# maomaomi1/Mean-Field-Multi-Agent-Reinforcement-Learning

Measured on NVIDIA B200. Metric: battle agent-steps/sec incl. obs+mean-action, higher is better.
Workload: dtype f32

## Files before the change

mean-field-multi-agent-reinforcement-learning_b200/csrc/battle_kernels.cuh:

```cuda
#pragma once
#include <cuda_runtime.h>
#include <stdint.h>

#include "battle_types.h"
#include "rng.cuh"

namespace mfmarl {

__device__ __forceinline__ int pos_x(int p) { return p & 0xFFFF; }
__device__ __forceinline__ int pos_y(int p) { return (p >> 16) & 0xFFFF; }
__device__ __forceinline__ int pack_pos(int x, int y) { return (x & 0xFFFF) | (y << 16); }
__device__ __forceinline__ uint32_t st_dead(uint32_t s) { return s & 1u; }
__device__ __forceinline__ uint32_t st_op(uint32_t s) { return (s >> 8) & 0xFFu; }
__device__ __forceinline__ uint32_t st_act(uint32_t s) { return (s >> 16) & 0xFFu; }
__device__ __forceinline__ uint32_t st_with_op(uint32_t s, uint32_t op) { return (s & ~0xFF00u) | (op << 8); }
__device__ __forceinline__ uint32_t make_state(uint32_t dead, uint32_t op, uint32_t act) {
    return dead | (op << 8) | (act << 16);
}

__device__ __forceinline__ int block_scan_flags2(bool fa, bool fb, int *s_warp, int &total) {
    const unsigned ba = __ballot_sync(0xFFFFFFFFu, fa), bb = __ballot_sync(0xFFFFFFFFu, fb);
    const int lane = threadIdx.x & 31, w = threadIdx.x >> 5;
    if (lane == 0) s_warp[w] = __popc(ba) | (__popc(bb) << 16);
    __syncthreads();
// ... 33 lines not shown
    R.hp10 = ((W + 2 * kPad) * (H + 2 * kPad) * 2 + 15) & ~15;
    R.mini = R.hp10 + 4 * 2 * cap;
    R.total = (R.mini + 4 * 2 * kViewCells + 15) & ~15;
    return R;
}

__device__ __forceinline__ void build_obs_record(const BattleParams &P, const BattleState &S, int e, uint16_t *s_pg, int *s_cnt) {
    const int tid = threadIdx.x, nt = blockDim.x, W = P.W, cap = P.cap, PW = W + 2 * kPad;
    const ObsRecord R = obs_record_layout(P.W, P.H, cap);
    unsigned char *rec = S.obs_record + (size_t)e * R.total;
    const size_t ebase = (size_t)e * 2 * cap;
    for (int c = tid; c < R.hp10 / 16; c += nt) ((uint4 *)s_pg)[c] = ((const uint4 *)S.grid_template)[c];
    for (int c = tid; c < 2 * kViewCells; c += nt) s_cnt[c] = 0;
    const int n0 = S.num[e * 2], n1 = S.num[e * 2 + 1];
    __syncthreads();
    const uint8_t *lut = S.mini_lut;
    float *hp10 = (float *)(rec + R.hp10);
    for (int s = tid; s < 2 * cap; s += nt) {
        const int gg = s >= cap, i = s - gg * cap;
        if (i >= (gg ? n1 : n0)) continue;
        const int p = S.pos[ebase + s], x = pos_x(p), y = pos_y(p);
        atomicAdd(&s_cnt[gg * kViewCells + lut[W + y] + lut[x]], 1);
        if (!st_dead(S.state[ebase + s])) {
            s_pg[(y + kPad) * PW + x + kPad] = (uint16_t)(((2 + gg) << 14) | s);
            hp10[s] = __fdiv_rn(S.hp[ebase + s], P.hp);
        }
    }
    __syncthreads();
    for (int c = tid; c < R.hp10 / 16; c += nt) ((uint4 *)rec)[c] = ((const uint4 *)s_pg)[c];
    float *mini = (float *)(rec + R.mini);
    for (int c = tid; c < 2 * kViewCells; c += nt) {
        const int tot = c >= kViewCells ? n1 : n0;
        mini[c] = tot > 0 ? __fdiv_rn((float)s_cnt[c], (float)tot) : 0.0f;
    }
}

__device__ __forceinline__ void place_from_template(const BattleParams &P, const BattleState &S, int e, int side) {
    const int cap = P.cap, n_action = P.n_move + P.n_attack;
    const size_t ebase = (size_t)e * 2 * cap;
    const int32_t *tpos = S.init_pos + (size_t)e * P.tmpl_stride;
    const int32_t *tnum = S.init_num + (P.tmpl_stride ? 2 * e : 0);
    for (int s = threadIdx.x; s < 2 * cap; s += blockDim.x) {
        const int g = s >= cap, i = s - g * cap, src = (side ? 1 - g : g) * cap + i;
        const bool live = i < tnum[side ? 1 - g : g];
        S.pos[ebase + s] = live ? tpos[src] : 0;
        S.hp[ebase + s] = P.hp;
        S.id[ebase + s] = live ? tpos[2 * cap + src] : 0;
        S.state[ebase + s] = make_state(0, OP_NULL, (uint32_t)n_action);
        S.next_rew[ebase + s] = P.step_reward;
        S.last_rew[ebase + s] = 0.0f;
    }
    if (threadIdx.x < 2) { S.num[e * 2 + threadIdx.x] = tnum[side ? 1 - threadIdx.x : threadIdx.x]; S.dead_ct[e * 2 + threadIdx.x] = 0; }
    if (threadIdx.x == 0) { S.step_ct[e] = 0; S.id_counter[e] = tnum[0] + tnum[1]; S.side[e] = side; }
}

__device__ __forceinline__ uint32_t minstd_jump(uint32_t s, uint32_t n) {
    const uint32_t pw[12] = {16807u, 282475249u, 984943658u, 1457850878u, 1137522503u, 1636807826u,
                             685118024u, 515204530u, 897054849u, 2038299453u, 1836275591u, 349037107u};
    uint64_t acc = s;
#pragma unroll
    for (int b = 0; b < 12; b++)
        if ((n >> b) & 1u) acc = (acc * pw[b]) % 2147483647ull;
    return (uint32_t)acc;
}

struct StepSmem {
    int pos, hp, nr, state, att, aux, mv, mvt, tag_a, tag_v, mvidx, scr0, scr1, grid, misc, total;
};
__host__ __device__ inline StepSmem step_smem_layout(int W, int H, int cap, int obs_cached) {
    StepSmem L;
    const int n = 2 * cap;
    int o = 0;
    L.pos = o;   o += 4 * n;
    L.hp = o;    o += 4 * n;
    L.nr = o;    o += 4 * n;
    L.state = o; o += 4 * n;
    L.att = o;   o += 4 * n;
    L.aux = o;   o += 4 * n;
    L.mv = o;    o += 4 * n;
    L.mvt = o;   o += 4 * n;
    L.scr0 = o;  o += 4 * n;
    L.scr1 = o;  o += 4 * n;
    L.tag_a = o; o += 2 * n;
    L.tag_v = o; o += 2 * n;
    L.mvidx = o; o += 2 * n;
    L.misc = o;  o += 4 * 128;
    L.grid = o;
    {
        int bytes = 4 * W * H;
        const int need = obs_record_layout(W, H, cap).hp10 + 4 * 2 * kViewCells;
        if (obs_cached && need > bytes) bytes = need;
        o += (bytes + 15) & ~15;
    }
    L.total = (o + 15) & ~15;
    return L;
}

enum { MISC_WARP = 0, MISC_N = 32, MISC_DEAD = 34, MISC_FLAG = 40, MISC_HIST = 64 };

enum : int { MV_FAIL = 0, MV_OK = 1, MV_WAIT = 2 };

__global__ void k_step(const __grid_constant__ BattleParams P, const BattleState S, const StepIO io) {
    extern __shared__ __align__(128) unsigned char smem_raw[];
    const StepSmem L = step_smem_layout(P.W, P.H, P.cap, P.obs_cached);
    int *s_pos = (int *)(smem_raw + L.pos);
    float *s_hp = (float *)(smem_raw + L.hp);
    float *s_nr = (float *)(smem_raw + L.nr);
    uint32_t *s_state = (uint32_t *)(smem_raw + L.state);
    uint32_t *s_att = (uint32_t *)(smem_raw + L.att);
    int *s_aux = (int *)(smem_raw + L.aux);
    uint32_t *s_mv = (uint32_t *)(smem_raw + L.mv);
    int *s_mvt = (int *)(smem_raw + L.mvt);
    int *s_scr0 = (int *)(smem_raw + L.scr0);
    int *s_scr1 = (int *)(smem_raw + L.scr1);
    uint16_t *s_tag_a = (uint16_t *)(smem_raw + L.tag_a);
    uint16_t *s_tag_v = (uint16_t *)(smem_raw + L.tag_v);
    uint16_t *s_mvidx = (uint16_t *)(smem_raw + L.mvidx);
    int *s_misc = (int *)(smem_raw + L.misc);
    uint32_t *s_grid = (uint32_t *)(smem_raw + L.grid);
    constexpr uint32_t kNoClaim = 0xFFFF0000u;

    const int e = blockIdx.x, tid = threadIdx.x, nt = blockDim.x;
    const int cap = P.cap, W = P.W, H = P.H, cells = W * H;
    const int n_action = P.n_move + P.n_attack;
    const size_t ebase = (size_t)e * 2 * cap;
    const int phases = io.phases;
    const int step_before = S.step_ct[e];

    if (tid < 2) { s_misc[MISC_N + tid] = S.num[e * 2 + tid]; s_misc[MISC_DEAD + tid] = S.dead_ct[e * 2 + tid]; }
    const uint8_t *walls = S.walls + (size_t)e * P.wall_stride;
    if ((cells & 3) == 0) {
        for (int c = tid; c < (cells >> 2); c += nt) {
            const uint32_t w4 = ((const uint32_t *)walls)[c];
            ((uint4 *)s_grid)[c] = make_uint4(kNoClaim | (w4 & 0xFFu), kNoClaim | ((w4 >> 8) & 0xFFu),
                                              kNoClaim | ((w4 >> 16) & 0xFFu), kNoClaim | (w4 >> 24));
        }
    } else {
        for (int c = tid; c < cells; c += nt) s_grid[c] = kNoClaim | walls[c];
    }
    __syncthreads();
    const int n0 = s_misc[MISC_N], n1 = s_misc[MISC_N + 1];
    for (int s = tid; s < 2 * cap; s += nt) {
        const int g = s >= cap, i = s - g * cap;
        if (i < (g ? n1 : n0)) {
            const int p = S.pos[ebase + s];
            uint32_t st = S.state[ebase + s];
            if ((phases & PH_SETACT) && ((io.setact_mask >> g) & 1)) {
                int a = io.actions[ebase + s];
                a = (a < 0 || a >= n_action) ? n_action : a;
                st = (st & 0xFF00FFFFu) | ((uint32_t)a << 16);
            }
            s_pos[s] = p; s_hp[s] = S.hp[ebase + s]; s_nr[s] = S.next_rew[ebase + s];
            s_state[s] = st;
            if (!st_dead(st)) s_grid[pos_y(p) * W + pos_x(p)] = kNoClaim | (uint32_t)(2 + s);
        }
        s_tag_a[s] = 0; s_tag_v[s] = 0; s_mvidx[s] = 0; s_scr0[s] = 0;
    }
    __syncthreads();

    int done = 0;
    if (phases & PH_STEP) {
        int nA = 0, nM = 0;
        const int n_pass = P.move_bands > 0 ? P.move_bands + 1 : 1;
        for (int pass = 0; pass < n_pass; pass++) {
            for (int gi = 0; gi < kGroups; gi++) {
                const int g = io.group_seq[gi];
                if (g < 0) continue;
                const int ng = g ? n1 : n0;
                for (int base = 0; base < ng; base += nt) {
                    const int i = base + tid, s = g * cap + i;
                    const bool valid = i < ng;
                    const int a = valid ? (int)st_act(s_state[s]) : n_action;
                    bool is_mv = valid && a < P.n_move;
                    const bool is_at = pass == 0 && valid && a >= P.n_move && a < n_action;
                    if (is_mv && n_pass > 1) {
                        const int x = pos_x(s_pos[s]), xr = x % P.band_width;
// ... 280 lines not shown
        __syncthreads();
        if (P.random_sides) {
            const uint4 r = philox4x32_10(make_uint4((uint32_t)episode, 0x51DEu, 0u, 0u), make_uint2(P.seed, (uint32_t)(P.env_base + e)));
            side = (int)(r.x & 1u);
        }
        place_from_template(P, S, e, side);
        if (tid == 0) S.episode[e] = episode;
    } else if (phases & PH_CLEAR) {
        for (int g = 0; g < kGroups; g++) {
            const int ng = g ? n1 : n0;
            int kept = 0;
            for (int base = 0; base < ng; base += nt) {
                const int i = base + tid, s = g * cap + i;
                const bool keep = i < ng && !st_dead(s_state[s]);
                const int my_id = keep ? S.id[ebase + s] : 0;
                int tot;
                const int p = block_scan_flag(keep, s_misc + MISC_WARP, tot);
                if (keep) {
                    const size_t d = ebase + (size_t)g * cap + kept + p;
                    S.pos[d] = s_pos[s]; S.hp[d] = s_hp[s]; S.id[d] = my_id;
                    S.state[d] = make_state(0, OP_NULL, st_act(s_state[s]));
                    S.last_rew[d] = s_nr[s];
                    S.next_rew[d] = P.step_reward;
                }
                kept += tot;
            }
            if (tid == 0) { S.num[e * 2 + g] = kept; S.dead_ct[e * 2 + g] = 0; }
        }
    } else if (phases & (PH_STEP | PH_SETACT)) {
        for (int s = tid; s < 2 * cap; s += nt) {
            const int g = s >= cap, i = s - g * cap;
            if (i < (g ? n1 : n0)) {
                S.pos[ebase + s] = s_pos[s]; S.hp[ebase + s] = s_hp[s];
                S.state[ebase + s] = s_state[s]; S.next_rew[ebase + s] = s_nr[s];
            }
        }
        if (tid < 2) S.dead_ct[e * 2 + tid] = s_misc[MISC_DEAD + tid];
    }
    if (io.mirror.pos != nullptr) {
        __syncthreads();
        for (int s = tid; s < 2 * cap; s += nt) {
            io.mirror.pos[s] = S.pos[ebase + s]; io.mirror.id[s] = S.id[ebase + s]; io.mirror.state[s] = S.state[ebase + s];
            io.mirror.hp[s] = S.hp[ebase + s]; io.mirror.next_rew[s] = S.next_rew[ebase + s];
            io.mirror.last_rew[s] = S.last_rew[ebase + s];
        }
        if (tid < 2) { io.mirror.head[tid] = S.num[e * 2 + tid]; io.mirror.head[2 + tid] = S.dead_ct[e * 2 + tid]; }
        if (tid == 0) { io.mirror.head[4] = done; io.mirror.head[5] = S.step_ct[e]; }
    }
    if (P.obs_cached && (phases & (PH_STEP | PH_CLEAR))) {
        __syncthreads();
        build_obs_record(P, S, e, (uint16_t *)(smem_raw + L.grid),
                         (int *)(smem_raw + L.grid + obs_record_layout(P.W, P.H, P.cap).hp10));
    }
}

__global__ void k_obs_record(const __grid_constant__ BattleParams P, const BattleState S) {
    extern __shared__ __align__(128) unsigned char smem_raw[];
    build_obs_record(P, S, blockIdx.x, (uint16_t *)smem_raw, (int *)(smem_raw + obs_record_layout(P.W, P.H, P.cap).hp10));
}

#ifndef MF_OBS_CHUNK
#define MF_OBS_CHUNK 8
#endif
constexpr int kObsChunk = MF_OBS_CHUNK;
constexpr int kObsThreads = 32 * kObsChunk, kObsWarps = kObsThreads / 32;
constexpr int kObsCtasPerSm = 16 / kObsChunk;
constexpr int kObsStageBytes = kObsChunk * kViewRow * 4;
constexpr int kViewRowBf16Bytes = kViewCells * 16;
constexpr int kObsPasses = (kViewCells + 31) / 32;
static_assert(kObsChunk == kObsWarps, "one warp composes one row of a chunk");

struct ObsSmem { int stage0, stage1, rec, hp10, mini, cnt, code, fxy, tmpl, record, total; };
constexpr int kObsMaxTile = kObsThreads;
__host__ __device__ inline bool obs_template_in_smem(int W, int H) { return (W + 2 * kPad) * (H + 2 * kPad) * 2 <= 8 * 1024; }
__host__ __device__ inline ObsSmem obs_smem_layout(int W, int H, int cap, int cached, int bf16 = 0) {
    ObsSmem L; int o = 0;
    const int stage_bytes = bf16 ? kObsChunk * kViewRowBf16Bytes : kObsStageBytes;
    L.stage0 = o; o += stage_bytes;
    L.stage1 = o; o += stage_bytes;
    L.rec = o;    o += 16 * kObsMaxTile;
    L.record = L.cnt = L.tmpl = 0;
    if (cached) {
        const ObsRecord R = obs_record_layout(W, H, cap);
        L.record = o; L.code = o + R.grid; L.hp10 = o + R.hp10; L.mini = o + R.mini; o += R.total;
        L.fxy = o;    o += 4 * (W + H);
        o = (o + 15) & ~15;
    } else {
        L.hp10 = o;   o += 4 * 2 * cap;
        L.mini = o;   o += 4 * 2 * kViewCells;
        L.cnt = o;    o += 4 * 2 * kViewCells;
        L.code = o;   o += (2 * (W + 2 * kPad) * (H + 2 * kPad) + 3) & ~3;
        L.fxy = o;    o += 4 * (W + H);
        o = (o + 15) & ~15;
        L.tmpl = o;   if (obs_template_in_smem(W, H)) o += (2 * (W + 2 * kPad) * (H + 2 * kPad) + 15) & ~15;
    }
    L.total = (o + 127) & ~127;
    return L;
}

__device__ __forceinline__ void bulk_store_s2g(void *gdst, const void *ssrc, uint32_t bytes) {
    const uint32_t saddr = (uint32_t)__cvta_generic_to_shared(ssrc);
    asm volatile("cp.async.bulk.global.shared::cta.bulk_group [%0], [%1], %2;"
                 :: "l"(gdst), "r"(saddr), "r"(bytes) : "memory");
}
__device__ __forceinline__ void bulk_commit() { asm volatile("cp.async.bulk.commit_group;" ::: "memory"); }
template <int N> __device__ __forceinline__ void bulk_wait_read() {
// ... 20 lines not shown
    extern __shared__ __align__(128) unsigned char smem_raw[];
    const ObsSmem L = obs_smem_layout(P.W, P.H, P.cap, CACHED, BF16);
    constexpr int kRowBytes = BF16 ? kViewRowBf16Bytes : kViewRow * 4;
    constexpr int kStageBytes = kObsChunk * kRowBytes;
    float *const s_stage0 = (float *)(smem_raw + L.stage0), *const s_stage1 = (float *)(smem_raw + L.stage1);
    int4 *s_rec = (int4 *)(smem_raw + L.rec);
    float *s_hp10 = (float *)(smem_raw + L.hp10);
    float *s_mini = (float *)(smem_raw + L.mini);
    int *s_cnt = (int *)(smem_raw + L.cnt);
    uint16_t *s_code = (uint16_t *)(smem_raw + L.code);
    float *s_fxy = (float *)(smem_raw + L.fxy);
    const bool tmpl_smem = !CACHED && obs_template_in_smem(P.W, P.H);
    const uint4 *s_tmpl = tmpl_smem ? (const uint4 *)(smem_raw + L.tmpl) : (const uint4 *)S.grid_template;
    const uint32_t rec_bytes = (uint32_t)obs_record_layout(P.W, P.H, P.cap).total;

    const int tid = threadIdx.x, lane = tid & 31, warp = tid >> 5;
    const int W = P.W, H = P.H, cap = P.cap;
    const int PW = W + 2 * kPad, pcells = PW * (H + 2 * kPad);
    const int FS = P.feature_size, emb = P.embedding_size, n_action = P.n_move + P.n_attack;
    const uint8_t *lut = S.mini_lut;

    constexpr int kDiscPasses = kObsDiscSlots / 32;
    int off[kDiscPasses], cell7[kDiscPasses];
#pragma unroll
    for (int it = 0; it < kDiscPasses; it++) {
        const int c = P.obs_cell[it * 32 + lane];
        const int vy = c / kView, vx = c - vy * kView;
        off[it] = c < kViewCells ? vy * PW + vx : 0;
        cell7[it] = c < kViewCells ? c * kChan : -1;
    }
    for (int i = tid; i < 2 * kStageBytes / 16; i += kObsThreads) ((uint4 *)s_stage0)[i] = make_uint4(0u, 0u, 0u, 0u);
    if (tmpl_smem)
        for (int c = tid; c < (pcells * 2 + 15) / 16; c += kObsThreads)
            ((uint4 *)(smem_raw + L.tmpl))[c] = ((const uint4 *)S.grid_template)[c];
    for (int i = tid; i < W + H; i += kObsThreads)
        s_fxy[i] = i < W ? __fdiv_rn((float)i, (float)W) : __fdiv_rn((float)(i - W), (float)H);

    int buf = 0;
    const int groups_per_env = io.group_mask == 3 ? 2 : 1;
    const int n_items = P.E * groups_per_env * io.tiles_per_group;
    __shared__ int s_next;
    if (tid == 0) s_next = atomicAdd(&S.obs_ticket[0], 1);
    for (;;) {
        __syncthreads();
        const int item = s_next;
        __syncthreads();
        if (item >= n_items) break;
        int next_ticket = 0;
        if (tid == 0) next_ticket = atomicAdd(&S.obs_ticket[0], 1);
        int t = item;
        const int tile = t % io.tiles_per_group; t /= io.tiles_per_group;
        int g, e;
        if (io.group_mask == 3) { g = t & 1; e = t >> 1; } else { g = io.group_mask >> 1; e = t; }
        const size_t ebase = (size_t)e * 2 * cap;
        const size_t gbase = ebase + (size_t)g * cap;
        const int a_begin = tile * io.tile_agents;
        int n0, n1, ng, a_end;
        if constexpr (CACHED) {
            {
                const unsigned char *src = S.obs_record + (size_t)e * rec_bytes;
                const uint32_t dst = (uint32_t)__cvta_generic_to_shared(smem_raw + L.record);
                for (uint32_t c = (uint32_t)tid * 16u; c < rec_bytes; c += kObsThreads * 16u)
                    asm volatile("cp.async.cg.shared.global [%0], [%1], 16;" :: "r"(dst + c), "l"(src + c) : "memory");
                asm volatile("cp.async.commit_group;" ::: "memory");
            }
            n0 = S.num[e * 2]; n1 = S.num[e * 2 + 1];
            int4 my_rec = make_int4(0, 0, 0, 0);
            if (tid < io.tile_agents && a_begin + tid < cap) {
                const size_t s = gbase + a_begin + tid;
                my_rec = make_int4(S.pos[s], S.id[s], (int)S.state[s], __float_as_int(S.last_rew[s]));
            }
            ng = g ? n1 : n0;
            a_end = min(ng, a_begin + io.tile_agents);
            if (tid < a_end - a_begin) s_rec[tid] = my_rec;
            asm volatile("cp.async.wait_all;" ::: "memory");
            if (a_begin >= ng) {
                if (tid == 0) s_next = next_ticket;
                continue;
            }
        } else {
        n0 = S.num[e * 2]; n1 = S.num[e * 2 + 1];
        constexpr int kPre = 4;
        int slot_pos[kPre]; uint32_t slot_state[kPre]; float slot_hp[kPre];
#pragma unroll
        for (int j = 0; j < kPre; j++) {
            const int s = tid + j * kObsThreads;
            slot_pos[j] = 0; slot_state[j] = 1u; slot_hp[j] = 0.0f;
            if (s < 2 * cap) { slot_pos[j] = S.pos[ebase + s]; slot_state[j] = S.state[ebase + s]; slot_hp[j] = S.hp[ebase + s]; }
        }
        int4 my_rec = make_int4(0, 0, 0, 0);
        if (tid < io.tile_agents && a_begin + tid < cap) {
            const size_t s = gbase + a_begin + tid;
            my_rec = make_int4(S.pos[s], S.id[s], (int)S.state[s], __float_as_int(S.last_rew[s]));
        }
        ng = g ? n1 : n0;
        if (a_begin >= ng) {
            if (tid == 0) s_next = next_ticket;
            continue;
        }
        a_end = min(ng, a_begin + io.tile_agents);

        for (int c = tid; c < (pcells * 2 + 15) / 16; c += kObsThreads) ((uint4 *)s_code)[c] = s_tmpl[c];
        for (int c = tid; c < 2 * kViewCells; c += kObsThreads) s_cnt[c] = 0;
        if (tid < a_end - a_begin) s_rec[tid] = my_rec;
        __syncthreads();
        auto place = [&](int s, int p, uint32_t st, float hp) {
// ... 238 lines not shown
```

mean-field-multi-agent-reinforcement-learning_b200/csrc/battle_types.h:

```cpp
#pragma once
#include <stdint.h>

namespace mfmarl {

constexpr int kGroups = 2;
constexpr int kMaxMoves = 32;
constexpr int kMaxAttacks = 32;
constexpr int kMaxActions = 64;
constexpr int kObsTicketRing = 8;
constexpr int kObsDiscSlots = 128;
constexpr int kView = 13, kViewCells = 169, kChan = 7, kViewRow = kViewCells * kChan;

enum : uint32_t { OP_KILL = 3, OP_COLLIDE = 6, OP_ATTACK = 7, OP_NULL = 11 };

enum RngMode : int {
    RNG_MINSTD = 0,
    RNG_PHILOX = 1,
    RNG_INJECT = 2,
};

enum StepPhase : int {
    PH_SETACT = 1,
    PH_STEP = 2,
    PH_EXPORT = 4,
    PH_CLEAR = 8,
    PH_AUTORESET = 16,
};

struct BattleParams {
    int E, W, H, cap;
    int env_base;
    int embedding_size;
    int n_move, n_attack;
    int view;
    int feature_size;
    int scale_w, scale_h;
    int wall_stride;
    int rng_mode;
    int max_steps;
    int tmpl_stride;
    int random_sides;
    int obs_cached;
    int move_bands;
    int band_width;
    uint32_t seed;
    float hp, damage, step_recover, kill_supply;
    float step_reward, kill_reward, dead_penalty, attack_penalty;
    float attack_bonus[kGroups];
    int8_t move_dx[kMaxMoves], move_dy[kMaxMoves];
    int8_t att_dx[kMaxAttacks], att_dy[kMaxAttacks];
    uint32_t disc[8];
    uint8_t obs_cell[kObsDiscSlots];
};

struct BattleState {
    int32_t *pos; float *hp; int32_t *id; uint32_t *state; float *next_rew; float *last_rew;
    int32_t *num; int32_t *dead_ct; uint32_t *rng; int32_t *step_ct; int32_t *id_counter;
    uint8_t *walls;
    uint16_t *grid_template;
    uint8_t *mini_lut;
    unsigned char *obs_record;
    unsigned long long *agent_steps;
    int32_t *obs_ticket;
    int32_t *init_pos; int32_t *init_num;
    int32_t *side;
    int32_t *episode;
};

struct StepMirror {
    int32_t *pos; int32_t *id; uint32_t *state; float *hp; float *next_rew; float *last_rew;
    int32_t *head;
};

struct StepIO {
    const int32_t *actions;
    const int32_t *attack_perm;
    float *reward;
    uint8_t *alive;
    float *mean_action;
    int32_t *done;
    int32_t *attack_events;
    StepMirror mirror;
    int phases;
    int setact_mask;
    int group_seq[kGroups];
};

struct ObsIO {
    float *view[kGroups];
    float *feature[kGroups];
    int env_stride;
    int group_mask;
    int tile_agents;
    int tiles_per_group;
    int debug;
};

constexpr int kLocalMaxTile = 128;
struct LocalMeanIO {
    float *out[kGroups];
    int group[kGroups];
    int W, H, cap, n_action;
    int tile;
    int n_offsets;
    int16_t delta[kViewCells];
};

}
```

mean-field-multi-agent-reinforcement-learning_b200/csrc/engine.cu:

```cuda
#include "engine.h"

#include <algorithm>
#include <cmath>
#include <cstdio>
#include <cstdlib>
#include <cstring>
#include <map>
#include <mutex>

#include "battle_kernels.cuh"

namespace mfmarl {

static thread_local std::string g_last_error;
void set_last_error(const std::string &msg) { g_last_error = msg; }
const char *last_error() { return g_last_error.c_str(); }

int report_fatal(const char *where, const std::exception &ex) {
    set_last_error(std::string(where) + ": " + ex.what());
    fprintf(stderr, "[magent/b200] fatal in %s: %s\n", where, ex.what());
    const char *mode = getenv("MAGENT_ERRORS");
    if (mode && strcmp(mode, "return") == 0) return -1;
    abort();
}
// ... 7 lines not shown
    const double delta = parity == 0 ? 0.5 : 0.0;
    for (int i = 0; i < width; i++)
        for (int j = 0; j < width; j++) {
            const double ax = std::fabs(j - center + delta), ay = std::fabs(i - center + delta);
            const double dis = std::sqrt(ax * ax + ay * ay);
            if (dis < radius + eps && dis > inner_radius - eps) {
                in[(size_t)i * width + j] = 1;
                dx.push_back(j - center);
                dy.push_back(i - center);
                count++;
            }
        }
}

void Engine::split_template() {
    if (!h_env_.empty()) return;
    h_env_.resize((size_t)P_.E);
    for (EnvTemplate &t : h_env_) {
        t.occ.assign(h_occ_.begin(), h_occ_.end());
        for (int g = 0; g < kGroups; g++) { t.pos[g] = h_tpos_[g]; t.id[g] = h_tid_[g]; }
        t.id_counter = h_id_counter_;
    }
}

void Engine::add_agents_per_env(int group, int n, const int *xs, const int *ys, int *n_added) {
    if (group < 0 || group >= kGroups) throw Fatal("invalid group handle in add_agents_per_env");
    if (stepped_) throw Fatal("add_agents_per_env after stepping is not supported (call reset first)");
    split_template();
    for (int e = 0; e < P_.E; e++) {
        EnvTemplate &t = h_env_[(size_t)e];
        int added = 0;
        for (int i = 0; i < n; i++) {
            const int x = xs[(size_t)e * n + i], y = ys[(size_t)e * n + i];
            if (x < 0 || y < 0 || x + 1 >= P_.W || y + 1 >= P_.H) continue;
            const size_t c = (size_t)y * P_.W + x;
            if (t.occ[c] != 0) continue;
            t.occ[c] = 2;
            t.pos[group].push_back(x | (y << 16));
            t.id[group].push_back(t.id_counter++);
            added++;
        }
        if (n_added) n_added[e] = added;
    }
    placement_dirty_ = true;
}

struct Engine::LateRecords {
    std::vector<int32_t> pos, id; std::vector<float> hp, nr, lr; std::vector<uint32_t> state;
    int num[2], dead[2];
};


static int round_up(int v, int m) { return (v + m - 1) / m * m; }

static void raise_dynamic_smem(const void *func, int bytes, int device) {
    static std::mutex mu;
    static std::map<std::pair<const void *, int>, int> granted;
    std::lock_guard<std::mutex> lock(mu);
    int &cur = granted[std::make_pair(func, device)];
    if (bytes <= cur) return;
    if (bytes > 227 * 1024)
        throw Fatal("geometry needs " + std::to_string(bytes) + " B of shared memory per CTA (limit 232448): map or capacity too large");
    MF_CUDA(cudaFuncSetAttribute(func, cudaFuncAttributeMaxDynamicSharedMemorySize, bytes));
    MF_CUDA(cudaFuncSetAttribute(func, cudaFuncAttributePreferredSharedMemoryCarveout, cudaSharedmemCarveoutMaxShared));
    cur = bytes;
}

Engine::Engine(const EngineConfig &cfg) : cfg_(cfg) {
    int ndev = 0;
    cudaError_t err = cudaGetDeviceCount(&ndev);
    if (err != cudaSuccess || ndev == 0)
        throw Fatal(std::string("no CUDA device: the battle engine has no CPU fallback (") +
                    cudaGetErrorString(err) + ")");
    if (cfg.device >= 0) MF_CUDA(cudaSetDevice(cfg.device));
    MF_CUDA(cudaGetDevice(&device_));
    MF_CUDA(cudaDeviceGetAttribute(&n_sm_, cudaDevAttrMultiProcessorCount, device_));

    if (cfg.n_envs < 1 || cfg.width < 3 || cfg.height < 3 || cfg.width > 4096 || cfg.height > 4096)
        throw Fatal("invalid engine config (n_envs / map size)");

    view_ = CircleRange(cfg.type.view_radius, 0.0f, 1);
    attack_ = CircleRange(cfg.type.attack_radius, 0.5f, 1);
    move_ = CircleRange(cfg.type.speed, 0.0f, 1);
    if (view_.width != kView)
        throw Fatal("view range " + std::to_string(view_.width) + "x" + std::to_string(view_.width) +
                    " unsupported: the observation kernel is specialised for the 13x13 battle view");
    if (move_.count > kMaxMoves || attack_.count > kMaxAttacks || move_.count + attack_.count > 32)
        throw Fatal("move/attack range too large (at most 32 actions)");

    P_.E = cfg.n_envs; P_.W = cfg.width; P_.H = cfg.height;
    P_.env_base = cfg.env_base;
    P_.embedding_size = cfg.embedding_size;
    P_.n_move = move_.count; P_.n_attack = attack_.count;
    P_.view = kView;
    P_.feature_size = cfg.embedding_size + P_.n_move + P_.n_attack + 1 + 2;
    P_.scale_w = (cfg.width + kView - 1) / kView;
    P_.scale_h = (cfg.height + kView - 1) / kView;
    P_.wall_stride = 0;
    P_.rng_mode = cfg.rng_mode; P_.max_steps = cfg.max_steps; P_.seed = cfg.seed;
    {
        const char *env = getenv("MFMARL_OBS_CACHED");
        const int want = cfg.obs_cached >= 0 ? cfg.obs_cached : (env ? atoi(env) : -1);
        P_.obs_cached = want >= 0 ? (want != 0) : (round_up(cfg.capacity, 4) >= 256);
    }
    P_.move_bands = 0; P_.band_width = cfg.width;
    if (cfg.width * cfg.height > 99 * 99) {
// ... 5 lines not shown
    P_.kill_reward = cfg.type.kill_reward; P_.dead_penalty = cfg.type.dead_penalty;
    P_.attack_penalty = cfg.type.attack_penalty;
    for (int g = 0; g < kGroups; g++) P_.attack_bonus[g] = cfg.attack_bonus[g];
    for (int i = 0; i < move_.count; i++) { P_.move_dx[i] = (int8_t)move_.dx[i]; P_.move_dy[i] = (int8_t)move_.dy[i]; }
    for (int i = 0; i < attack_.count; i++) { P_.att_dx[i] = (int8_t)attack_.dx[i]; P_.att_dy[i] = (int8_t)attack_.dy[i]; }
    memset(P_.disc, 0, sizeof(P_.disc));
    for (int c = 0; c < kViewCells; c++)
        if (view_.in[c]) P_.disc[c >> 5] |= 1u << (c & 31);
    {
        memset(P_.obs_cell, 255, sizeof(P_.obs_cell));
        const int passes = kObsDiscSlots / 32;
        std::vector<int> left;
        for (int c = 0; c < kViewCells; c++) {
            if (!view_.in[c]) continue;
            bool placed = false;
            for (int p = 0; p < passes && !placed; p++)
                if (P_.obs_cell[p * 32 + (c & 31)] == 255) { P_.obs_cell[p * 32 + (c & 31)] = (uint8_t)c; placed = true; }
            if (!placed) left.push_back(c);
        }
        for (int c : left) {
            int slot = -1;
            for (int s = 0; s < kObsDiscSlots && slot < 0; s++) if (P_.obs_cell[s] == 255) slot = s;
            if (slot < 0) throw Fatal("view disc has more than 128 cells: k_obs lane schedule too small");
            P_.obs_cell[slot] = (uint8_t)c;
        }
    }

    const size_t E = (size_t)P_.E;
    MF_CUDA(cudaMalloc(&S_.num, E * 2 * sizeof(int32_t)));
    MF_CUDA(cudaMalloc(&S_.dead_ct, E * 2 * sizeof(int32_t)));
    MF_CUDA(cudaMalloc(&S_.rng, E * sizeof(uint32_t)));
    MF_CUDA(cudaMalloc(&S_.step_ct, E * sizeof(int32_t)));
    MF_CUDA(cudaMalloc(&S_.id_counter, E * sizeof(int32_t)));
    MF_CUDA(cudaMalloc(&S_.walls, (size_t)P_.W * P_.H));
    MF_CUDA(cudaMalloc(&S_.init_num, E * 2 * sizeof(int32_t)));
    MF_CUDA(cudaMalloc(&S_.side, E * sizeof(int32_t)));
    MF_CUDA(cudaMalloc(&S_.episode, E * sizeof(int32_t)));
    MF_CUDA(cudaMemset(S_.side, 0, E * sizeof(int32_t)));
    MF_CUDA(cudaMemset(S_.episode, 0, E * sizeof(int32_t)));
    P_.tmpl_stride = 0; P_.random_sides = cfg.random_sides != 0;
    MF_CUDA(cudaMalloc(&S_.grid_template, grid_template_bytes()));
    {
        if ((P_.H - 1) / P_.scale_h * kView + (P_.W - 1) / P_.scale_w > 255) throw Fatal("minimap table overflow");
        std::vector<uint8_t> lut((size_t)P_.W + P_.H);
        for (int x = 0; x < P_.W; x++) lut[x] = (uint8_t)(x / P_.scale_w);
        for (int y = 0; y < P_.H; y++) lut[(size_t)P_.W + y] = (uint8_t)((y / P_.scale_h) * kView);
        MF_CUDA(cudaMalloc(&S_.mini_lut, lut.size()));
        MF_CUDA(cudaMemcpy(S_.mini_lut, lut.data(), lut.size(), cudaMemcpyHostToDevice));
    }
    MF_CUDA(cudaMalloc(&S_.agent_steps, E * sizeof(unsigned long long)));
    MF_CUDA(cudaMemset(S_.agent_steps, 0, E * sizeof(unsigned long long)));
    MF_CUDA(cudaMalloc(&S_.obs_ticket, 2 * kObsTicketRing * sizeof(int32_t)));
    MF_CUDA(cudaMemset(S_.obs_ticket, 0, 2 * kObsTicketRing * sizeof(int32_t)));
    MF_CUDA(cudaMemset(S_.num, 0, E * 2 * sizeof(int32_t)));
    MF_CUDA(cudaMemset(S_.dead_ct, 0, E * 2 * sizeof(int32_t)));
    MF_CUDA(cudaMemset(S_.step_ct, 0, E * sizeof(int32_t)));
    MF_CUDA(cudaMemset(S_.id_counter, 0, E * sizeof(int32_t)));
    h_num_.assign(E * 2, 0);
#ifdef MF_PROFILE_BUILD
    { const char *dbg = getenv("MFMARL_OBS_DEBUG"); obs_debug_ = dbg ? atoi(dbg) : 0; }
#endif
    { const char *lim = getenv("MFMARL_OBS_GRID"); obs_grid_limit_ = lim ? atoi(lim) : 0; }
    set_seed(cfg.seed);
    alloc_state(std::max(4, round_up(cfg.capacity, 4)));
    reset();
}

Engine::~Engine() {
    free_state();
    cudaFree(S_.num); cudaFree(S_.dead_ct); cudaFree(S_.rng); cudaFree(S_.step_ct);
    cudaFree(S_.id_counter); cudaFree(S_.walls); cudaFree(S_.init_num); cudaFree(S_.agent_steps); cudaFree(S_.obs_ticket); cudaFree(S_.mini_lut); cudaFree(S_.grid_template);
    cudaFree(S_.side); cudaFree(S_.episode);
}

size_t Engine::grid_template_bytes() const {
    const size_t cells = (size_t)(P_.W + 2 * (kView / 2)) * (P_.H + 2 * (kView / 2));
    return (cells * 2 + 15) / 16 * 16;
}

void Engine::alloc_state(int cap) {
    if (2 * cap > 0x3FFF) throw Fatal("capacity too large for the 14-bit slot field of the occupancy grid");
    P_.cap = cap;
    const size_t n = slots();
    MF_CUDA(cudaMalloc(&S_.pos, n * 4)); MF_CUDA(cudaMalloc(&S_.hp, n * 4));
    MF_CUDA(cudaMalloc(&S_.id, n * 4)); MF_CUDA(cudaMalloc(&S_.state, n * 4));
    MF_CUDA(cudaMalloc(&S_.next_rew, n * 4)); MF_CUDA(cudaMalloc(&S_.last_rew, n * 4));
    MF_CUDA(cudaMalloc(&S_.init_pos, (size_t)P_.E * 4 * cap * 4));
    S_.obs_record = nullptr;
    if (P_.obs_cached) {
        const size_t bytes = (size_t)P_.E * obs_record_layout(P_.W, P_.H, cap).total;
        MF_CUDA(cudaMalloc(&S_.obs_record, bytes));
        MF_CUDA(cudaMemset(S_.obs_record, 0, bytes));
    }
    MF_CUDA(cudaMemset(S_.pos, 0, n * 4)); MF_CUDA(cudaMemset(S_.hp, 0, n * 4));
    MF_CUDA(cudaMemset(S_.id, 0, n * 4)); MF_CUDA(cudaMemset(S_.state, 0, n * 4));
    MF_CUDA(cudaMemset(S_.next_rew, 0, n * 4)); MF_CUDA(cudaMemset(S_.last_rew, 0, n * 4));
}

void Engine::free_state() {
    cudaFree(S_.pos); cudaFree(S_.hp); cudaFree(S_.id); cudaFree(S_.state);
    cudaFree(S_.next_rew); cudaFree(S_.last_rew); cudaFree(S_.init_pos); cudaFree(S_.obs_record);
    S_.obs_record = nullptr;
    S_.pos = nullptr; S_.hp = nullptr; S_.id = nullptr; S_.state = nullptr;
    S_.next_rew = S_.last_rew = nullptr; S_.init_pos = nullptr;
}

void Engine::set_seed(unsigned long seed) {
    unsigned long s = seed % 2147483647ul;
    std::vector<uint32_t> h((size_t)P_.E, (uint32_t)(s == 0 ? 1 : s));
    MF_CUDA(cudaMemcpy(S_.rng, h.data(), h.size() * 4, cudaMemcpyHostToDevice));
    P_.seed = (uint32_t)seed;
}

void Engine::reset() {
    const int W = P_.W, H = P_.H;
    h_walls_.assign((size_t)W * H, 0);
    for (int i = 0; i < W; i++) { h_walls_[i] = 1; h_walls_[(size_t)(H - 1) * W + i] = 1; }
    for (int i = 0; i < H; i++) { h_walls_[(size_t)i * W] = 1; h_walls_[(size_t)i * W + W - 1] = 1; }
    h_occ_.assign(h_walls_.begin(), h_walls_.end());
    for (int g = 0; g < kGroups; g++) { h_tpos_[g].clear(); h_tid_[g].clear(); }
    h_id_counter_ = 0;
    h_env_.clear();
    placement_dirty_ = true;
    stepped_ = false;
// ... 203 lines not shown
    float *v[kGroups] = {d_view, d_view + (size_t)P_.cap * kViewRow};
    float *f[kGroups] = {d_feature, d_feature + (size_t)P_.cap * P_.feature_size};
    observe_groups(v, f, 2 * P_.cap, group_mask, st);
}

void Engine::observe_groups(float *const d_view[kGroups], float *const d_feature[kGroups], int env_stride,
                            int group_mask, cudaStream_t st, bool bf16) {
    commit(st);
    if (group_mask < 1 || group_mask > 3) throw Fatal("observe: bad group mask");
    ObsIO io;
    for (int g = 0; g < kGroups; g++) {
        io.view[g] = d_view[g]; io.feature[g] = d_feature[g];
        if (((group_mask >> g) & 1) && (!d_view[g] || !d_feature[g])) throw Fatal("observe: null output buffer");
        if (((group_mask >> g) & 1) && ((uintptr_t)d_view[g] & 15)) throw Fatal("observe: view buffer must be 16-byte aligned");
    }
    io.env_stride = env_stride; io.group_mask = group_mask;
    io.debug = obs_debug_;
    const ObsSmem L = obs_smem_layout(P_.W, P_.H, P_.cap, P_.obs_cached, bf16);
    void (*kern)(const BattleParams, const BattleState, const ObsIO) =
        P_.obs_cached ? (bf16 ? k_obs<true, true> : k_obs<true, false>) : (bf16 ? k_obs<false, true> : k_obs<false, false>);
    raise_dynamic_smem((const void *)kern, L.total, device_);
    int &ctas_per_sm = obs_ctas_per_sm_[bf16 ? 1 : 0];
    if (obs_attr_[bf16 ? 1 : 0] != L.total) {
        MF_CUDA(cudaOccupancyMaxActiveBlocksPerMultiprocessor(&ctas_per_sm, kern, kObsThreads, L.total));
        obs_attr_[bf16 ? 1 : 0] = L.total;
    }
    size_t ctas = (size_t)std::max(1, ctas_per_sm) * n_sm_;
    if (cfg_.concurrent_step_envs > 0) {
        const int step_smem = step_smem_layout(P_.W, P_.H, P_.cap, P_.obs_cached).total + 1024;
        const int sm_smem = 227 * 1024, obs_smem = L.total + 1024;
        const int fit_beside_full = (sm_smem - ctas_per_sm * obs_smem) / step_smem;
        if (fit_beside_full < 1 && ctas_per_sm > 1) {
            const int per_freed_slot = std::max(1, (sm_smem - (ctas_per_sm - 1) * obs_smem) / step_smem);
            const size_t reserve = ((size_t)cfg_.concurrent_step_envs + per_freed_slot - 1) / per_freed_slot;
            ctas = ctas > reserve + (size_t)n_sm_ ? ctas - reserve : (size_t)n_sm_;
        }
    }
    int want_tile = cfg_.obs_tile_agents;
    if (want_tile <= 0 && P_.obs_cached) {
        want_tile = 64;
    } else if (want_tile <= 0) {
        want_tile = std::min(256, std::max(64, P_.cap));
        const size_t groups = (size_t)P_.E * (group_mask == 3 ? 2 : 1);
        while (want_tile > 128 && groups * ((P_.cap + want_tile - 1) / want_tile) < 3 * ctas) want_tile /= 2;
        while (want_tile > kObsChunk && groups * ((P_.cap + want_tile - 1) / want_tile) < ctas / 8) want_tile /= 2;
    }
    io.tile_agents = std::min(kObsMaxTile, std::max(kObsChunk, round_up(want_tile, kObsChunk)));
    io.tiles_per_group = (P_.cap + io.tile_agents - 1) / io.tile_agents;
    const size_t items = (size_t)P_.E * (group_mask == 3 ? 2 : 1) * io.tiles_per_group;
    unsigned grid = (unsigned)std::min<size_t>(items, ctas);
    if (obs_grid_limit_ > 0) grid = std::min(grid, (unsigned)obs_grid_limit_);
    BattleState S = S_;
    S.obs_ticket += 2 * (obs_launches_++ % kObsTicketRing);
    kern<<<grid, kObsThreads, L.total, st>>>(P_, S, io);
    MF_CUDA(cudaGetLastError());
}

void Engine::step(const StepIO &io, cudaStream_t st) {
    commit(st);
    const StepSmem L = step_smem_layout(P_.W, P_.H, P_.cap, P_.obs_cached);
    raise_dynamic_smem((const void *)k_step, L.total, device_);
    int threads = cfg_.step_threads > 0 ? cfg_.step_threads : std::min(1024, std::max(64, P_.cap));
    if (cfg_.step_threads <= 0 && P_.E <= n_sm_ / 2) threads = std::max(threads, 256);
    threads = round_up(threads, 32);
    k_step<<<P_.E, threads, L.total, st>>>(P_, S_, io);
    MF_CUDA(cudaGetLastError());
    if (io.phases & (PH_STEP | PH_CLEAR | PH_SETACT)) stepped_ = true;
}

void Engine::mean_action(const int32_t *d_actions, const int32_t *d_num, float *d_out, int rows, int cap,
                         int n_action, cudaStream_t st) {
    if (n_action > 32) throw Fatal("mean_action: at most 32 actions");
    const int warps_per_block = 8;
    const int blocks = (rows + warps_per_block - 1) / warps_per_block;
    k_mean_action<<<blocks, warps_per_block * 32, 0, st>>>(d_actions, d_num, d_out, rows, cap, n_action);
    MF_CUDA(cudaGetLastError());
}

void Engine::local_mean_action(double radius, float *const out[kGroups], cudaStream_t st) {
    const double view_radius = cfg_.type.view_radius;
    if (!(radius > 0.0 && radius <= view_radius)) {
        char msg[160];
        snprintf(msg, sizeof(msg), "local_mean_action: radius %g outside (0, view_radius = %g]", radius, view_radius);
        throw Fatal(msg);
    }
    int group_mask = 0;
    for (int g = 0; g < kGroups; g++) {
        if (!out[g]) continue;
        if ((uintptr_t)out[g] & 15) throw Fatal("local_mean_action: output buffer must be 16-byte aligned");
        group_mask |= 1 << g;
    }
    commit(st);
    if (!group_mask) return;
    const float r = (float)radius;
    auto it = local_discs_.find(r);
    if (it == local_discs_.end()) {
        const CircleRange disc(r, 0.0f, 1);
        if (disc.center > kPad) throw Fatal("local_mean_action: disc wider than the grid margin");
        LocalMeanIO t{};
        const int PW = P_.W + 2 * kPad;
        for (int k = 0; k < disc.count; k++)
            if (disc.dx[k] != 0 || disc.dy[k] != 0) t.delta[t.n_offsets++] = (int16_t)(disc.dy[k] * PW + disc.dx[k]);
        it = local_discs_.emplace(r, t).first;
    }
    LocalMeanIO io = it->second;
    io.W = P_.W; io.H = P_.H; io.cap = P_.cap; io.n_action = n_action();
    io.tile = std::min(kLocalMaxTile, round_up(P_.cap, 32));
    int ng = 0;
    for (int g = 0; g < kGroups; g++) {
        io.out[g] = out[g];
        if ((group_mask >> g) & 1) io.group[ng++] = g;
    }
    const LocalMeanSmem L = local_mean_smem_layout(P_.W, P_.H, io.tile, io.n_action);
    raise_dynamic_smem((const void *)k_local_mean_action, L.total, device_);
    const dim3 grid((unsigned)P_.E, (unsigned)((P_.cap + io.tile - 1) / io.tile), (unsigned)ng);
    k_local_mean_action<<<grid, io.tile, L.total, st>>>(io, S_);
    MF_CUDA(cudaGetLastError());
}
// ... 3 lines not shown
```

mean-field-multi-agent-reinforcement-learning_b200/csrc/engine.h:

```cpp
#pragma once
#include <cuda_runtime.h>

#include <map>
#include <memory>
#include <stdexcept>
#include <string>
#include <vector>

#include "battle_types.h"

namespace mfmarl {

struct Fatal : std::runtime_error {
    using std::runtime_error::runtime_error;
};

#define MF_CUDA(expr)                                                                              \
    do {                                                                                           \
        cudaError_t err__ = (expr);                                                                \
        if (err__ != cudaSuccess)                                                                  \
            throw ::mfmarl::Fatal(std::string(#expr) + " failed: " + cudaGetErrorString(err__) +   \
                                  " (" __FILE__ ":" + std::to_string(__LINE__) + ")");             \
    } while (0)

// ... 38 lines not shown

    void observe(float *d_view, float *d_feature, int group_mask, cudaStream_t st);
    void observe_groups(float *const d_view[kGroups], float *const d_feature[kGroups], int env_stride, int group_mask,
                        cudaStream_t st, bool bf16 = false);
    void step(const StepIO &io, cudaStream_t st);
    static void mean_action(const int32_t *d_actions, const int32_t *d_num, float *d_out, int rows,
                            int cap, int n_action, cudaStream_t st);
    void local_mean_action(double radius, float *const out[kGroups], cudaStream_t st);

    void restore_state(const int32_t *pos, const int32_t *id, const uint32_t *state, const float *hp, const float *next_rew,
                       const float *last_rew, const int32_t *num, const int32_t *dead_ct, cudaStream_t st);

    void commit(cudaStream_t st);
    void download_num(cudaStream_t st);
    const BattleParams &params() const { return P_; }
    void set_rng_mode(int mode) { P_.rng_mode = mode; }
    void mark_stepped() { stepped_ = true; }
    const std::vector<unsigned char> &host_walls() const { return h_walls_; }
    uint32_t pull_rng0();
    void push_rng0(uint32_t s);
    bool cell_blank_for_placement(int x, int y);
    const BattleState &state() const { return S_; }
    int cap() const { return P_.cap; }
    int n_envs() const { return P_.E; }
    int n_action() const { return P_.n_move + P_.n_attack; }
    int host_num(int env, int group) const { return h_num_[env * 2 + group]; }
    void set_host_num(int env, int group, int n) { h_num_[env * 2 + group] = n; }
    bool placement_pending() const { return placement_dirty_; }
    size_t slots() const { return (size_t)P_.E * 2 * P_.cap; }
    const CircleRange &view_range() const { return view_; }
    const CircleRange &attack_range() const { return attack_; }
    const CircleRange &move_range() const { return move_; }

private:
    void alloc_state(int cap);
    size_t grid_template_bytes() const;
    void free_state();
    void grow(int need_cap);
    void late_add_sync_down();
    void late_add_sync_up();
    void rebuild_obs_records(cudaStream_t st);

    struct LateRecords;
    std::unique_ptr<LateRecords> late_;

    EngineConfig cfg_;
    BattleParams P_{};
    BattleState S_{};
    CircleRange view_, attack_, move_;
    int device_ = 0;
    int n_sm_ = 148;
    int obs_attr_[2] = {-1, -1};
    unsigned obs_launches_ = 0;
    int obs_ctas_per_sm_[2] = {2, 2};
    int obs_grid_limit_ = 0;
    int obs_debug_ = 0;
    std::map<float, LocalMeanIO> local_discs_;

    std::vector<unsigned char> h_walls_;
    std::vector<int> h_occ_;
    std::vector<int> h_tpos_[kGroups], h_tid_[kGroups];
    int h_id_counter_ = 0;
    struct EnvTemplate { std::vector<unsigned char> occ; std::vector<int> pos[kGroups], id[kGroups]; int id_counter = 0; };
    std::vector<EnvTemplate> h_env_;
    void split_template();
    bool placement_dirty_ = true;
    bool stepped_ = false;
    std::vector<int> h_num_;
};

void set_last_error(const std::string &msg);
const char *last_error();
int report_fatal(const char *where, const std::exception &ex);

}
```

Baseline: 1.605 billion.

## Overlap observation kernel with step kernel via programmatic dependent launch and per-env flags

```diff
diff --git a/mean-field-multi-agent-reinforcement-learning_b200/csrc/battle_kernels.cuh b/mean-field-multi-agent-reinforcement-learning_b200/csrc/battle_kernels.cuh
--- a/mean-field-multi-agent-reinforcement-learning_b200/csrc/battle_kernels.cuh
+++ b/mean-field-multi-agent-reinforcement-learning_b200/csrc/battle_kernels.cuh
@@ -109,6 +109,15 @@
     }
     if (threadIdx.x < 2) { S.num[e * 2 + threadIdx.x] = tnum[side ? 1 - threadIdx.x : threadIdx.x]; S.dead_ct[e * 2 + threadIdx.x] = 0; }
     if (threadIdx.x == 0) { S.step_ct[e] = 0; S.id_counter[e] = tnum[0] + tnum[1]; S.side[e] = side; }
+}
+
+__device__ __forceinline__ int ld_acquire_gpu(const int32_t *p) {
+    int v;
+    asm volatile("ld.acquire.gpu.global.b32 %0, [%1];" : "=r"(v) : "l"(p) : "memory");
+    return v;
+}
+__device__ __forceinline__ void st_release_gpu(int32_t *p, int v) {
+    asm volatile("st.release.gpu.global.b32 [%0], %1;" :: "l"(p), "r"(v) : "memory");
 }
 
 __device__ __forceinline__ uint32_t minstd_jump(uint32_t s, uint32_t n) {
@@ -179,6 +188,7 @@
 
     const int e = blockIdx.x, tid = threadIdx.x, nt = blockDim.x;
     const int cap = P.cap, W = P.W, H = P.H, cells = W * H;
+    asm volatile("griddepcontrol.launch_dependents;" ::: "memory");
     const int n_action = P.n_move + P.n_attack;
     const size_t ebase = (size_t)e * 2 * cap;
     const int phases = io.phases;
@@ -565,6 +575,10 @@
         build_obs_record(P, S, e, (uint16_t *)(smem_raw + L.grid),
                          (int *)(smem_raw + L.grid + obs_record_layout(P.W, P.H, P.cap).hp10));
     }
+    if (io.ready) {
+        __syncthreads();
+        if (tid == 0) { __threadfence(); st_release_gpu(io.ready + e, io.ready_seq); }
+    }
 }
 
 __global__ void k_obs_record(const __grid_constant__ BattleParams P, const BattleState S) {
@@ -691,6 +705,13 @@
         const int tile = t % io.tiles_per_group; t /= io.tiles_per_group;
         int g, e;
         if (io.group_mask == 3) { g = t & 1; e = t >> 1; } else { g = io.group_mask >> 1; e = t; }
+        if constexpr (CACHED) {
+            if (io.ready) {
+                if (tid == 0)
+                    while (ld_acquire_gpu(io.ready + e) - io.ready_seq < 0) __nanosleep(64);
+                __syncthreads();
+            }
+        }
         const size_t ebase = (size_t)e * 2 * cap;
         const size_t gbase = ebase + (size_t)g * cap;
         const int a_begin = tile * io.tile_agents;
diff --git a/mean-field-multi-agent-reinforcement-learning_b200/csrc/battle_types.h b/mean-field-multi-agent-reinforcement-learning_b200/csrc/battle_types.h
--- a/mean-field-multi-agent-reinforcement-learning_b200/csrc/battle_types.h
+++ b/mean-field-multi-agent-reinforcement-learning_b200/csrc/battle_types.h
@@ -62,6 +62,7 @@
     unsigned char *obs_record;
     unsigned long long *agent_steps;
     int32_t *obs_ticket;
+    int32_t *step_ready;
     int32_t *init_pos; int32_t *init_num;
     int32_t *side;
     int32_t *episode;
@@ -84,6 +85,8 @@
     int phases;
     int setact_mask;
     int group_seq[kGroups];
+    int32_t *ready;
+    int ready_seq;
 };
 
 struct ObsIO {
@@ -94,6 +97,8 @@
     int tile_agents;
     int tiles_per_group;
     int debug;
+    const int32_t *ready;
+    int ready_seq;
 };
 
 constexpr int kLocalMaxTile = 128;
diff --git a/mean-field-multi-agent-reinforcement-learning_b200/csrc/engine.cu b/mean-field-multi-agent-reinforcement-learning_b200/csrc/engine.cu
--- a/mean-field-multi-agent-reinforcement-learning_b200/csrc/engine.cu
+++ b/mean-field-multi-agent-reinforcement-learning_b200/csrc/engine.cu
@@ -83,6 +83,12 @@
 
 
 static int round_up(int v, int m) { return (v + m - 1) / m * m; }
+
+static bool capturing(cudaStream_t st) {
+    cudaStreamCaptureStatus cs = cudaStreamCaptureStatusNone;
+    MF_CUDA(cudaStreamIsCapturing(st, &cs));
+    return cs != cudaStreamCaptureStatusNone;
+}
 
 static void raise_dynamic_smem(const void *func, int bytes, int device) {
     static std::mutex mu;
@@ -194,6 +200,8 @@
     MF_CUDA(cudaMemset(S_.agent_steps, 0, E * sizeof(unsigned long long)));
     MF_CUDA(cudaMalloc(&S_.obs_ticket, 2 * kObsTicketRing * sizeof(int32_t)));
     MF_CUDA(cudaMemset(S_.obs_ticket, 0, 2 * kObsTicketRing * sizeof(int32_t)));
+    MF_CUDA(cudaMalloc(&S_.step_ready, E * sizeof(int32_t)));
+    MF_CUDA(cudaMemset(S_.step_ready, 0, E * sizeof(int32_t)));
     MF_CUDA(cudaMemset(S_.num, 0, E * 2 * sizeof(int32_t)));
     MF_CUDA(cudaMemset(S_.dead_ct, 0, E * 2 * sizeof(int32_t)));
     MF_CUDA(cudaMemset(S_.step_ct, 0, E * sizeof(int32_t)));
@@ -211,7 +219,7 @@
 Engine::~Engine() {
     free_state();
     cudaFree(S_.num); cudaFree(S_.dead_ct); cudaFree(S_.rng); cudaFree(S_.step_ct);
-    cudaFree(S_.id_counter); cudaFree(S_.walls); cudaFree(S_.init_num); cudaFree(S_.agent_steps); cudaFree(S_.obs_ticket); cudaFree(S_.mini_lut); cudaFree(S_.grid_template);
+    cudaFree(S_.id_counter); cudaFree(S_.walls); cudaFree(S_.init_num); cudaFree(S_.agent_steps); cudaFree(S_.obs_ticket); cudaFree(S_.step_ready); cudaFree(S_.mini_lut); cudaFree(S_.grid_template);
     cudaFree(S_.side); cudaFree(S_.episode);
 }
 
@@ -521,8 +529,17 @@
     if (obs_grid_limit_ > 0) grid = std::min(grid, (unsigned)obs_grid_limit_);
     BattleState S = S_;
     S.obs_ticket += 2 * (obs_launches_++ % kObsTicketRing);
-    kern<<<grid, kObsThreads, L.total, st>>>(P_, S, io);
-    MF_CUDA(cudaGetLastError());
+    io.ready = nullptr; io.ready_seq = 0;
+    cudaLaunchAttribute attr[1];
+    cudaLaunchConfig_t cfg = {};
+    cfg.gridDim = dim3(grid); cfg.blockDim = dim3(kObsThreads); cfg.dynamicSmemBytes = L.total; cfg.stream = st;
+    if (P_.obs_cached && ready_seq_ != 0 && st == ready_stream_ && !capturing(st)) {
+        io.ready = S_.step_ready; io.ready_seq = ready_seq_;
+        attr[0].id = cudaLaunchAttributeProgrammaticStreamSerialization;
+        attr[0].val.programmaticStreamSerializationAllowed = 1;
+        cfg.attrs = attr; cfg.numAttrs = 1;
+    }
+    MF_CUDA(cudaLaunchKernelEx(&cfg, kern, P_, S, io));
 }
 
 void Engine::step(const StepIO &io, cudaStream_t st) {
@@ -532,7 +549,14 @@
     int threads = cfg_.step_threads > 0 ? cfg_.step_threads : std::min(1024, std::max(64, P_.cap));
     if (cfg_.step_threads <= 0 && P_.E <= n_sm_ / 2) threads = std::max(threads, 256);
     threads = round_up(threads, 32);
-    k_step<<<P_.E, threads, L.total, st>>>(P_, S_, io);
+    StepIO sio = io;
+    ready_seq_ = 0;
+    if (!capturing(st)) {
+        if (++step_launches_ <= 0) step_launches_ = 1;
+        sio.ready = S_.step_ready; sio.ready_seq = ready_seq_ = step_launches_;
+        ready_stream_ = st;
+    }
+    k_step<<<P_.E, threads, L.total, st>>>(P_, S_, sio);
     MF_CUDA(cudaGetLastError());
     if (io.phases & (PH_STEP | PH_CLEAR | PH_SETACT)) stepped_ = true;
 }
diff --git a/mean-field-multi-agent-reinforcement-learning_b200/csrc/engine.h b/mean-field-multi-agent-reinforcement-learning_b200/csrc/engine.h
--- a/mean-field-multi-agent-reinforcement-learning_b200/csrc/engine.h
+++ b/mean-field-multi-agent-reinforcement-learning_b200/csrc/engine.h
@@ -114,6 +114,9 @@
     int n_sm_ = 148;
     int obs_attr_[2] = {-1, -1};
     unsigned obs_launches_ = 0;
+    int step_launches_ = 0;
+    int ready_seq_ = 0;
+    cudaStream_t ready_stream_ = nullptr;
     int obs_ctas_per_sm_[2] = {2, 2};
     int obs_grid_limit_ = 0;
     int obs_debug_ = 0;
```

Result: no change. 1.596 billion, median of 6 (-0.5%).
